# SymbioticLab/Oobleck

Hardware: AMD Instinct MI355X
Metric: tokens/sec (whole node) GPT-2 1F1B (higher is better)
Workload: dtype bf16; 1 GPU; gpt2.yaml GPT-2-small 1F1B, global microbatch 128x1024 tokens, bf16; model=gpt2, global_batch=128, seq_len=1024, parallelism=pp1dp1

## Files before the change

### include/oobleck_stage.h

```cpp
#ifndef OOBLECK_STAGE_H
#define OOBLECK_STAGE_H

#include <stdint.h>

#ifdef __cplusplus
extern "C" {
#endif

enum {
  OB_KIND_EMBED = 0,
  OB_KIND_BLOCK = 1,
  OB_KIND_FINAL = 2
};

typedef struct ob_layer* ob_layer_t;

typedef struct {
  int32_t kind;
  int32_t n_embd;
  int32_t n_head;
  int32_t n_positions;
  int32_t vocab_size;
  int32_t max_batch;
  int32_t seq_len;
// ... 103 lines not shown
int ob_dropout_add_f32(uint64_t seed, int32_t layer_id, int32_t site,
                       uint64_t tick, float p, const void* t, const void* res,
                       void* y, int64_t n, void* stream);
int ob_dropout_add_bf16(uint64_t seed, int32_t layer_id, int32_t site,
                        uint64_t tick, float p, const void* t,
                        const void* res, void* y, int64_t n, void* stream);
int ob_dropout_scale_colsum_f32(uint64_t seed, int32_t layer_id, int32_t site,
                                uint64_t tick, float p, const void* dy,
                                void* dm, void* db, int64_t M, int64_t N,
                                void* stream);
int ob_dropout_scale_colsum_bf16(uint64_t seed, int32_t layer_id, int32_t site,
                                 uint64_t tick, float p, const void* dy,
                                 void* dm, void* db, int64_t M, int64_t N,
                                 void* stream);

int ob_gemm_bf16(int transA, int transB, int64_t M, int64_t N, int64_t K,
                 float alpha, const void* A, int64_t lda,
                 int64_t strideA1, int64_t strideA2,
                 const void* B, int64_t ldb,
                 int64_t strideB1, int64_t strideB2,
                 float beta, void* C, int64_t ldc,
                 int64_t strideC1, int64_t strideC2,
                 int64_t n1, int64_t n2,
                 const void* bias, const void* residual, int out_kind,
                 int splitk, void* stream);

int ob_flash_fwd_nt_bf16(const void* qkv, void* O, void* lse, int64_t B,
                         int64_t Sq, int64_t H, int64_t nh, float scale,
                         void* stream);
int ob_flash_bwd_nt_bf16(const void* qkv, const void* dO, const void* lse,
                         const void* D, void* dqkv, void* dbias_qkv,
                         int64_t B, int64_t Sq, int64_t H, int64_t nh,
                         float scale, void* stream);

int ob_f32_to_bf16(const void* x, void* y, int64_t n, void* stream);
int ob_f32_to_bf16_t(const void* x, void* y, int64_t rows, int64_t cols,
                     void* stream);
int ob_bf16_to_f32(const void* x, void* y, int64_t n, void* stream);

void ob_profile_enable(int on);
void ob_profile_reset(void);
int ob_profile_read(int fam, double* total_ms, long long* count);

const char* ob_last_error(void);

const char* ob_build_arch(void);

#ifdef __cplusplus
}
#endif
#endif
```

### oobleck_amd/_ext.py

```python
from __future__ import annotations

import ctypes
import pathlib

_LIB = None
SO_PATH = pathlib.Path(__file__).resolve().parent / "libob_stage.so"


class ObLayerDesc(ctypes.Structure):
    _fields_ = [
        ("kind", ctypes.c_int32),
        ("n_embd", ctypes.c_int32),
        ("n_head", ctypes.c_int32),
        ("n_positions", ctypes.c_int32),
        ("vocab_size", ctypes.c_int32),
        ("max_batch", ctypes.c_int32),
        ("seq_len", ctypes.c_int32),
        ("n_slots", ctypes.c_int32),
        ("dtype", ctypes.c_int32),
    ]


class ObDropoutDesc(ctypes.Structure):
    _fields_ = [
# ... 82 lines not shown
    lib.ob_flash_fwd_bf16.argtypes = [vp, vp, vp, vp, i64, i64, i64, i64,
                                      f32, vp]
    lib.ob_transpose_bf16_b.argtypes = [vp, vp, i64, i64, i64, i64, i64,
                                        i64, i64, vp]
    lib.ob_layernorm_fwd_bf16.argtypes = [vp, vp, vp, vp, vp, vp, i64, i64,
                                          f32, vp]
    lib.ob_layernorm_bwd_bf16.argtypes = [vp, vp, vp, vp, vp, vp, vp, vp,
                                          i64, i64, i32, vp]
    lib.ob_colsum_bf16.argtypes = [vp, vp, i64, i64, vp]
    lib.ob_layernorm_fwd_copy_bf16.argtypes = [vp, vp, vp, vp, vp, vp, vp,
                                               i64, i64, f32, vp]
    lib.ob_layernorm_bwd_res_bf16.argtypes = [vp, vp, vp, vp, vp, vp, vp, vp,
                                              vp, vp, vp, i64, i64, vp]
    lib.ob_gelu_bwd_colsum_bf16.argtypes = [vp, vp, vp, vp, i64, i64, vp]
    lib.ob_gemm_lt.argtypes = [i32, i32, i64, i64, i64, f32, vp, i64, vp,
                               i64, f32, vp, i64, i32, vp]
    lib.ob_gemm_bf16_nt_8ph.argtypes = [vp, vp, vp, vp, vp, i64, i64, i64,
                                        i64, i64, i64, i64, i64, i64, i64,
                                        i64, i64, i64, i64, f32, f32, i32,
                                        i32, vp, i64]
    lib.ob_profile_enable.argtypes = [i32]
    lib.ob_profile_enable.restype = None
    lib.ob_profile_reset.argtypes = []
    lib.ob_profile_reset.restype = None
    lib.ob_profile_read.argtypes = [i32, ctypes.POINTER(ctypes.c_double),
                                    ctypes.POINTER(ctypes.c_longlong)]
    lib.ob_flash_dsum_bf16.argtypes = [vp, vp, vp, i64, i64, i64, i64, vp]
    lib.ob_flash_bwd_bf16.argtypes = [vp, vp, vp, vp, vp, vp, vp, vp, i64,
                                      i64, i64, i64, f32, vp]
    lib.ob_flash_fwd_nt_bf16.argtypes = [vp, vp, vp, i64, i64, i64, i64,
                                         f32, vp]
    lib.ob_flash_bwd_nt_bf16.argtypes = [vp, vp, vp, vp, vp, vp, i64, i64,
                                         i64, i64, f32, vp]
    return lib


def get_ext(build_if_missing: bool = True) -> ctypes.CDLL:
    global _LIB
    if _LIB is not None:
        return _LIB
    if not SO_PATH.exists():
        if build_if_missing:
            from .build import build
            try:
                build()
            except Exception as e:
                raise RuntimeError(
                    f"oobleck_amd: HIP extension missing and build failed: {e}. "
                    "The hot path has no fallback — run __graft_entry__.build().") from e
        else:
            raise RuntimeError(
                "oobleck_amd: HIP extension libob_stage.so is missing. "
                "The hot path has no fallback — run __graft_entry__.build().")
    _LIB = _configure(ctypes.CDLL(str(SO_PATH)))
    return _LIB


def check(rc: int, what: str = "") -> None:
    if rc != 0:
        err = get_ext().ob_last_error().decode()
        raise RuntimeError(f"oobleck_amd extension error in {what}: {err}")
```

### oobleck_amd/build.py

```python
from __future__ import annotations

import pathlib
import subprocess

PKG_DIR = pathlib.Path(__file__).resolve().parent
SO_PATH = PKG_DIR / "libob_stage.so"
SOURCES = [PKG_DIR / "csrc" / "ob_kernels.hip",
           PKG_DIR / "csrc" / "ob_kernels_bf16.hip",
           PKG_DIR / "csrc" / "ob_flash_bf16.hip",
           PKG_DIR / "csrc" / "ob_blaslt.hip",
           PKG_DIR / "csrc" / "ob_optim.hip",
           PKG_DIR / "csrc" / "ob_dropout.hip",
           PKG_DIR / "csrc" / "ob_layer.hip"]
HEADERS = [PKG_DIR.parent / "include" / "oobleck_stage.h",
           PKG_DIR / "csrc" / "ob_internal.h",
           PKG_DIR / "csrc" / "ob_philox.h"]


def needs_rebuild() -> bool:
    if not SO_PATH.exists():
        return True
    so_mtime = SO_PATH.stat().st_mtime
    return any(p.stat().st_mtime > so_mtime for p in SOURCES + HEADERS)


def build(force: bool = False) -> pathlib.Path:
    if force or needs_rebuild():
        cmd = ["hipcc", "--offload-arch=gfx950", "-O3", "-std=c++17", "-fPIC",
               "-shared"] + [str(s) for s in SOURCES] + \
              ["-L/opt/rocm/lib", "-lhipblaslt", "-o", str(SO_PATH)]
        subprocess.run(cmd, check=True, capture_output=True, text=True)
    return SO_PATH


if __name__ == "__main__":
    print(build(force=True))
```

### oobleck_amd/csrc/ob_flash_bf16.hip

```cpp
#include "ob_internal.h"

#include <cmath>

using f32x16 = __attribute__((ext_vector_type(16))) float;
using bf16x8 = __attribute__((ext_vector_type(8))) __bf16;
using bf16x4 = __attribute__((ext_vector_type(4))) __bf16;

static inline hipStream_t S(void* s) { return reinterpret_cast<hipStream_t>(s); }

__device__ __forceinline__ float bf2f(__bf16 h) { return (float)h; }

__device__ __forceinline__ unsigned bf_bits(__bf16 h) {
  return (unsigned)__builtin_bit_cast(unsigned short, h);
}
__device__ __forceinline__ __bf16 bits_bf(unsigned u) {
  return __builtin_bit_cast(__bf16, (unsigned short)(u & 0xffffu));
}

__device__ __forceinline__ __bf16 bf_extract(const uint4& v, int j) {
  const unsigned word = (j < 2) ? v.x : (j < 4) ? v.y : (j < 6) ? v.z : v.w;
  return bits_bf((j & 1) ? (word >> 16) : word);
}

__device__ __forceinline__ uint4 bf_pack8(const float* v) {
  uint4 o;
  o.x = bf_bits((__bf16)v[0]) | (bf_bits((__bf16)v[1]) << 16);
  o.y = bf_bits((__bf16)v[2]) | (bf_bits((__bf16)v[3]) << 16);
  o.z = bf_bits((__bf16)v[4]) | (bf_bits((__bf16)v[5]) << 16);
  o.w = bf_bits((__bf16)v[6]) | (bf_bits((__bf16)v[7]) << 16);
  return o;
}

__device__ __forceinline__ unsigned bf_pk2(float a, float b) {
// ... 19 lines not shown
  fr.x = x0;
  fr.y = x1;
  fr.z = y0;
  fr.w = y1;
  return __builtin_bit_cast(bf16x8, fr);
}

__device__ __forceinline__ int acc_row(int r, int kh) {
  return (r & 3) + 8 * (r >> 2) + 4 * kh;
}

__device__ __forceinline__ int nt_key(int row) {
  return (((row >> 1) & 1) << 2) | ((row >> 2) & 3);
}
__device__ __forceinline__ int nt_off(int row, int ch) {
  return row * 64 + ((ch ^ nt_key(row)) << 3);
}
__device__ __forceinline__ bf16x8 nt_tr_frag(const __bf16* tile, int lane,
                                             int r0, int dhalf) {
  typedef __attribute__((address_space(3))) bf16x4 lds_bf16x4;
  const int i = lane & 15;
  const int row = r0 + (i >> 2);
  const int ch = 4 * dhalf + 2 * ((lane >> 4) & 1) + ((i >> 1) & 1);
  const int sub = 4 * (i & 1);
  const bf16x4 lo = __builtin_amdgcn_ds_read_tr16_b64_v4bf16(
      (lds_bf16x4*)(tile + nt_off(row, ch) + sub));
  const bf16x4 hi = __builtin_amdgcn_ds_read_tr16_b64_v4bf16(
      (lds_bf16x4*)(tile + nt_off(row + 4, ch) + sub));
  return __builtin_shufflevector(lo, hi, 0, 1, 2, 3, 4, 5, 6, 7);
}

__global__ __launch_bounds__(256, 3) void k_flash_fwd_nt(
    const __bf16* __restrict__ qkv, __bf16* __restrict__ Obase,
    float* __restrict__ lse, int Sq, int H, int nh, float scale) {
  __shared__ __attribute__((aligned(16))) __bf16 kbuf[2][64 * 64];
  __shared__ __attribute__((aligned(16))) __bf16 vbuf[2][64 * 64];
  __shared__ float bcast[128];
  const int z = blockIdx.z;
  const int b = z / nh, h = z % nh;
  const int64_t qoff = (int64_t)b * Sq * 3 * H + h * 64;
  const __bf16* Qp = qkv + qoff;
  const __bf16* Kp = Qp + H;
  const __bf16* Vp = Qp + 2 * H;
  __bf16* Op = Obase + (int64_t)b * Sq * H + h * 64;
  float* lsep = lse + (int64_t)z * Sq;

  const int tid = threadIdx.x;
  const int lane = tid & 63;
  const int w = tid >> 6;
  const int il = lane & 31, kh = lane >> 5;
  const int q0b = blockIdx.x * 128;
  const int q0 = q0b + w * 32;
  const int myq = q0 + il;

  const int sr0 = tid >> 3, sr1 = sr0 + 32, sc = tid & 7;
  const int so0 = nt_off(sr0, sc), so1 = nt_off(sr1, sc);
  auto stage = [&](int buf, int kv0) {
    *reinterpret_cast<bf16x8*>(&kbuf[buf][so0]) =
        *reinterpret_cast<const bf16x8*>(
            Kp + (int64_t)(kv0 + sr0) * 3 * H + sc * 8);
    *reinterpret_cast<bf16x8*>(&kbuf[buf][so1]) =
        *reinterpret_cast<const bf16x8*>(
            Kp + (int64_t)(kv0 + sr1) * 3 * H + sc * 8);
    *reinterpret_cast<bf16x8*>(&vbuf[buf][so0]) =
        *reinterpret_cast<const bf16x8*>(
            Vp + (int64_t)(kv0 + sr0) * 3 * H + sc * 8);
    *reinterpret_cast<bf16x8*>(&vbuf[buf][so1]) =
        *reinterpret_cast<const bf16x8*>(
            Vp + (int64_t)(kv0 + sr1) * 3 * H + sc * 8);
  };

  bf16x8 qf[4];
#pragma unroll
  for (int s = 0; s < 4; ++s)
    qf[s] = *reinterpret_cast<const bf16x8*>(
        Qp + (int64_t)myq * 3 * H + s * 16 + kh * 8);

  const int ntiles = (q0b + 128) / 64;
  stage(0, 0);
  __syncthreads();

  f32x16 o0 = {}, o1 = {};
  float m = -INFINITY, l = 0.f;
  for (int kvt = 0; kvt < ntiles; ++kvt) {
    const int kv0 = kvt * 64;
    if (kvt + 1 < ntiles) stage((kvt + 1) & 1, kv0 + 64);
    const bool active = kv0 <= q0 + 31;
    if (active) {
      const __bf16* kb = kbuf[kvt & 1];
      const __bf16* vb = vbuf[kvt & 1];
      f32x16 sacc0 = {}, sacc1 = {};
#pragma unroll
      for (int s = 0; s < 4; ++s) {
        const int ch = (s * 2 + kh);
        const bf16x8 ka =
            *reinterpret_cast<const bf16x8*>(&kb[nt_off(il, ch)]);
        const bf16x8 kb2 =
            *reinterpret_cast<const bf16x8*>(&kb[nt_off(32 + il, ch)]);
        sacc0 = __builtin_amdgcn_mfma_f32_32x32x16_bf16(ka, qf[s], sacc0, 0,
                                                        0, 0);
        sacc1 = __builtin_amdgcn_mfma_f32_32x32x16_bf16(kb2, qf[s], sacc1,
                                                        0, 0, 0);
      }
      float sv[32];
      if (kv0 + 63 < q0) {
#pragma unroll
        for (int r = 0; r < 16; ++r) {
          sv[r] = sacc0[r] * scale;
          sv[16 + r] = sacc1[r] * scale;
        }
      } else {
#pragma unroll
        for (int r = 0; r < 16; ++r) {
          const int kvr = kv0 + (r & 3) + 8 * (r >> 2) + 4 * kh;
          sv[r] = (kvr <= myq) ? sacc0[r] * scale : -INFINITY;
          sv[16 + r] = (kvr + 32 <= myq) ? sacc1[r] * scale : -INFINITY;
        }
      }
      float mx[8];
#pragma unroll
// ... 27 lines not shown
                   ((ps[4] + ps[5]) + (ps[6] + ps[7]));
      psum += __shfl_xor(psum, 32, 64);
      l += psum;
#pragma unroll
      for (int t = 0; t < 4; ++t) {
        const bf16x8 pa = bf_dance(sv + t * 8);
        const bf16x8 v0f = nt_tr_frag(vb, lane, t * 16 + kh * 8, 0);
        const bf16x8 v1f = nt_tr_frag(vb, lane, t * 16 + kh * 8, 1);
        o0 = __builtin_amdgcn_mfma_f32_32x32x16_bf16(pa, v0f, o0, 0, 0, 0);
        o1 = __builtin_amdgcn_mfma_f32_32x32x16_bf16(pa, v1f, o1, 0, 0, 0);
      }
    }
    __syncthreads();
  }

  if (kh == 0) {
    bcast[w * 32 + il] = 1.f / l;
    lsep[myq] = m + __logf(l);
  }
#pragma unroll
  for (int r = 0; r < 16; ++r) {
    const int row = (r & 3) + 8 * (r >> 2) + 4 * kh;
    const float inv = bcast[w * 32 + row];
    Op[(int64_t)(q0 + row) * H + il] = (__bf16)(o0[r] * inv);
    Op[(int64_t)(q0 + row) * H + 32 + il] = (__bf16)(o1[r] * inv);
  }
}

extern "C" int ob_flash_fwd_nt_bf16(const void* qkv, void* O, void* lse,
                                    int64_t B, int64_t Sq, int64_t H,
                                    int64_t nh, float scale, void* stream) {
  if (H / nh != 64) return ob_fail("flash_fwd_nt: head_dim must be 64");
  if (Sq % 128) return ob_fail("flash_fwd_nt: S must be a multiple of 128");
  dim3 grid((unsigned)(Sq / 128), 1, (unsigned)(B * nh));
  k_flash_fwd_nt<<<grid, 256, 0, S(stream)>>>(
      (const __bf16*)qkv, (__bf16*)O, (float*)lse, (int)Sq, (int)H, (int)nh,
      scale);
  OB_LAUNCH_CHECK();
  return 0;
}

__global__ __launch_bounds__(256, 3) void k_flash_bwd_dkdv_nt(
    const __bf16* __restrict__ qkv, const __bf16* __restrict__ dO,
    const float* __restrict__ lse, const float* __restrict__ D,
    __bf16* __restrict__ dqkv, float* __restrict__ dbias, int Sq, int H,
    int nh, float scale) {
  __shared__ float xch[2][2][32 * 32];
  __shared__ __attribute__((aligned(16))) __bf16 qbuf[2][32 * 64];
  __shared__ __attribute__((aligned(16))) __bf16 obuf[2][32 * 64];
  __shared__ float red[4 * 64];
  const int z = blockIdx.z;
  const int b = z / nh, h = z % nh;
  const int64_t base = (int64_t)b * Sq * 3 * H + h * 64;
  const __bf16* Qp = qkv + base;
  const __bf16* Kp = Qp + H;
  const __bf16* Vp = Qp + 2 * H;
  const __bf16* dOp = dO + (int64_t)b * Sq * H + h * 64;
  const float* lsep = lse + (int64_t)z * Sq;
  const float* Dp = D + (int64_t)z * Sq;

  const int tid = threadIdx.x;
  const int lane = tid & 63;
  const int w = tid >> 6;
  const int pair = w >> 1, role = w & 1;
  const int il = lane & 31, kh = lane >> 5;
  const int kv0 = blockIdx.x * 64 + pair * 32;
  const int mykv = kv0 + il;

  const __bf16* KV = role ? Vp : Kp;
  bf16x8 of[4];
#pragma unroll
  for (int s = 0; s < 4; ++s)
    of[s] = *reinterpret_cast<const bf16x8*>(
        KV + (int64_t)mykv * 3 * H + s * 16 + kh * 8);

  const int srow = tid >> 3, schunk = tid & 7;
  const int so = nt_off(srow, schunk);
  auto stage = [&](int buf, int q0s) {
    *reinterpret_cast<bf16x8*>(&qbuf[buf][so]) =
        *reinterpret_cast<const bf16x8*>(
            Qp + (int64_t)(q0s + srow) * 3 * H + schunk * 8);
    *reinterpret_cast<bf16x8*>(&obuf[buf][so]) =
        *reinterpret_cast<const bf16x8*>(
            dOp + (int64_t)(q0s + srow) * H + schunk * 8);
  };

  f32x16 acc0 = {}, acc1 = {};
  const int nqt = Sq / 32;
  const int qt0 = (blockIdx.x * 64) / 32;
  stage(qt0 & 1, qt0 * 32);
  __syncthreads();

  for (int qt = qt0; qt < nqt; ++qt) {
    const int q0 = qt * 32;
    if (qt + 1 < nqt) stage((qt + 1) & 1, q0 + 32);
    const __bf16* ab = role ? obuf[qt & 1] : qbuf[qt & 1];
    const __bf16* bb = role ? qbuf[qt & 1] : obuf[qt & 1];
    const bf16x8 b00 = nt_tr_frag(bb, lane, kh * 8, 0);
    const bf16x8 b01 = nt_tr_frag(bb, lane, kh * 8, 1);
    const bf16x8 b10 = nt_tr_frag(bb, lane, 16 + kh * 8, 0);
    const bf16x8 b11 = nt_tr_frag(bb, lane, 16 + kh * 8, 1);
    f32x16 own = {};
#pragma unroll
    for (int s = 0; s < 4; ++s) {
      const int ch = s * 2 + kh;
      const bf16x8 af =
          *reinterpret_cast<const bf16x8*>(&ab[nt_off(il, ch)]);
      own = __builtin_amdgcn_mfma_f32_32x32x16_bf16(af, of[s], own, 0, 0,
                                                    0);
    }
    float pv[16];
    float* ptile = xch[qt & 1][pair];
    if (role == 0) {
      const float lse_t = lsep[q0 + il];
#pragma unroll
      for (int r = 0; r < 16; ++r) {
        const int qoff = acc_row(r, kh);
        const bool ok = q0 + qoff >= mykv;
        const float lse_q = __shfl(lse_t, qoff, 64);
        pv[r] = ok ? __expf(own[r] * scale - lse_q) : 0.f;
        ptile[qoff * 32 + il] = pv[r];
      }
    }
    __syncthreads();
    if (role == 1) {
      const float d_t = Dp[q0 + il];
#pragma unroll
      for (int r = 0; r < 16; ++r) {
// ... 12 lines not shown
    }
  }

  __bf16* outp = dqkv + base + (role ? H : 2 * H);
  const float os = role ? scale : 1.f;
#pragma unroll
  for (int r = 0; r < 16; ++r) {
    const int kv = kv0 + acc_row(r, kh);
    outp[(int64_t)kv * 3 * H + il] = (__bf16)(os * acc0[r]);
    outp[(int64_t)kv * 3 * H + 32 + il] = (__bf16)(os * acc1[r]);
  }
  if (dbias) {
    float c0 = 0.f, c1 = 0.f;
#pragma unroll
    for (int r = 0; r < 16; ++r) {
      c0 += os * acc0[r];
      c1 += os * acc1[r];
    }
    c0 += __shfl_xor(c0, 32, 64);
    c1 += __shfl_xor(c1, 32, 64);
    if (kh == 0) {
      red[w * 64 + il] = c0;
      red[w * 64 + 32 + il] = c1;
    }
    __syncthreads();
    if (tid < 128) {
      const int rl = tid >> 6, c = tid & 63;
      atomicAdd(dbias + (rl ? H : 2 * H) + h * 64 + c,
                red[rl * 64 + c] + red[(2 + rl) * 64 + c]);
    }
  }
}

__global__ __launch_bounds__(256, 3) void k_flash_bwd_dq_nt(
    const __bf16* __restrict__ qkv, const __bf16* __restrict__ dO,
    const float* __restrict__ lse, const float* __restrict__ D,
    __bf16* __restrict__ dqkv, float* __restrict__ dbias, int Sq, int H,
    int nh, float scale) {
  __shared__ __attribute__((aligned(16))) __bf16 kbuf[2][64 * 64];
  __shared__ __attribute__((aligned(16))) __bf16 vbuf[2][64 * 64];
  __shared__ float red[4 * 64];
  const int z = blockIdx.z;
  const int b = z / nh, h = z % nh;
  const int64_t base = (int64_t)b * Sq * 3 * H + h * 64;
  const __bf16* Qp = qkv + base;
  const __bf16* Kp = Qp + H;
  const __bf16* Vp = Qp + 2 * H;
  const __bf16* dOp = dO + (int64_t)b * Sq * H + h * 64;
  const float* lsep = lse + (int64_t)z * Sq;
  const float* Dp = D + (int64_t)z * Sq;

  const int tid = threadIdx.x;
  const int lane = tid & 63;
  const int w = tid >> 6;
  const int il = lane & 31, kh = lane >> 5;
  const int q0 = blockIdx.x * 128 + w * 32;
  const int myq = q0 + il;
  const float mylse = lsep[myq];
  const float myD = Dp[myq];

  bf16x8 qf[4], df[4];
#pragma unroll
  for (int s = 0; s < 4; ++s) {
    qf[s] = *reinterpret_cast<const bf16x8*>(
        Qp + (int64_t)myq * 3 * H + s * 16 + kh * 8);
    df[s] = *reinterpret_cast<const bf16x8*>(
        dOp + (int64_t)myq * H + s * 16 + kh * 8);
  }

  const int srow = tid >> 3, schunk = tid & 7;
  const int so0 = nt_off(srow, schunk), so1 = nt_off(srow + 32, schunk);
  auto stage = [&](int buf, int kv0) {
    *reinterpret_cast<bf16x8*>(&kbuf[buf][so0]) =
        *reinterpret_cast<const bf16x8*>(
            Kp + (int64_t)(kv0 + srow) * 3 * H + schunk * 8);
    *reinterpret_cast<bf16x8*>(&kbuf[buf][so1]) =
        *reinterpret_cast<const bf16x8*>(
            Kp + (int64_t)(kv0 + srow + 32) * 3 * H + schunk * 8);
    *reinterpret_cast<bf16x8*>(&vbuf[buf][so0]) =
        *reinterpret_cast<const bf16x8*>(
            Vp + (int64_t)(kv0 + srow) * 3 * H + schunk * 8);
    *reinterpret_cast<bf16x8*>(&vbuf[buf][so1]) =
        *reinterpret_cast<const bf16x8*>(
            Vp + (int64_t)(kv0 + srow + 32) * 3 * H + schunk * 8);
  };

  const int ntiles = (blockIdx.x * 128 + 128) / 64;
  stage(0, 0);
  __syncthreads();

  f32x16 dq0 = {}, dq1 = {};
  for (int kvt = 0; kvt < ntiles; ++kvt) {
    const int kv0 = kvt * 64;
    if (kvt + 1 < ntiles) stage((kvt + 1) & 1, kv0 + 64);
    const bool active = kv0 <= q0 + 31;
    if (active) {
      const __bf16* kb = kbuf[kvt & 1];
      const __bf16* vb = vbuf[kvt & 1];
      f32x16 s0 = {}, s1 = {}, p0 = {}, p1 = {};
#pragma unroll
      for (int s = 0; s < 4; ++s) {
        const int ch = s * 2 + kh;
        const bf16x8 ka =
            *reinterpret_cast<const bf16x8*>(&kb[nt_off(il, ch)]);
        const bf16x8 kb2 =
            *reinterpret_cast<const bf16x8*>(&kb[nt_off(32 + il, ch)]);
        const bf16x8 va =
            *reinterpret_cast<const bf16x8*>(&vb[nt_off(il, ch)]);
        const bf16x8 vb2 =
            *reinterpret_cast<const bf16x8*>(&vb[nt_off(32 + il, ch)]);
        s0 = __builtin_amdgcn_mfma_f32_32x32x16_bf16(ka, qf[s], s0, 0, 0, 0);
        s1 = __builtin_amdgcn_mfma_f32_32x32x16_bf16(kb2, qf[s], s1, 0, 0,
                                                     0);
        p0 = __builtin_amdgcn_mfma_f32_32x32x16_bf16(va, df[s], p0, 0, 0, 0);
        p1 = __builtin_amdgcn_mfma_f32_32x32x16_bf16(vb2, df[s], p1, 0, 0,
                                                     0);
      }
      float dsv[32];
#pragma unroll
      for (int r = 0; r < 16; ++r) {
        const int kv = kv0 + (r & 3) + 8 * (r >> 2) + 4 * kh;
        const bool ok0 = kv <= myq;
        const bool ok1 = kv + 32 <= myq;
        const float pa = ok0 ? __expf(s0[r] * scale - mylse) : 0.f;
        const float pb = ok1 ? __expf(s1[r] * scale - mylse) : 0.f;
        dsv[r] = ok0 ? pa * (p0[r] - myD) : 0.f;
        dsv[16 + r] = ok1 ? pb * (p1[r] - myD) : 0.f;
      }
// ... 5 lines not shown
        dq0 = __builtin_amdgcn_mfma_f32_32x32x16_bf16(da, kt0, dq0, 0, 0, 0);
        dq1 = __builtin_amdgcn_mfma_f32_32x32x16_bf16(da, kt1, dq1, 0, 0, 0);
      }
    }
    __syncthreads();
  }
  __bf16* dQp = dqkv + base;
#pragma unroll
  for (int r = 0; r < 16; ++r) {
    const int q = q0 + (r & 3) + 8 * (r >> 2) + 4 * kh;
    dQp[(int64_t)q * 3 * H + il] = (__bf16)(scale * dq0[r]);
    dQp[(int64_t)q * 3 * H + 32 + il] = (__bf16)(scale * dq1[r]);
  }
  if (dbias) {
    float c0 = 0.f, c1 = 0.f;
#pragma unroll
    for (int r = 0; r < 16; ++r) {
      c0 += scale * dq0[r];
      c1 += scale * dq1[r];
    }
    c0 += __shfl_xor(c0, 32, 64);
    c1 += __shfl_xor(c1, 32, 64);
    if (kh == 0) {
      red[w * 64 + il] = c0;
      red[w * 64 + 32 + il] = c1;
    }
    __syncthreads();
    if (tid < 64)
      atomicAdd(dbias + h * 64 + tid, (red[tid] + red[64 + tid]) +
                                          (red[128 + tid] + red[192 + tid]));
  }
}

extern "C" int ob_flash_bwd_nt_bf16(const void* qkv, const void* dO,
                                    const void* lse, const void* D,
                                    void* dqkv, void* dbias_qkv, int64_t B,
                                    int64_t Sq, int64_t H, int64_t nh,
                                    float scale, void* stream) {
  if (H / nh != 64) return ob_fail("flash_bwd_nt: head_dim must be 64");
  if (Sq % 128) return ob_fail("flash_bwd_nt: S must be a multiple of 128");
  dim3 gridp((unsigned)(Sq / 64), 1, (unsigned)(B * nh));
  k_flash_bwd_dkdv_nt<<<gridp, 256, 0, S(stream)>>>(
      (const __bf16*)qkv, (const __bf16*)dO, (const float*)lse,
      (const float*)D, (__bf16*)dqkv, (float*)dbias_qkv, (int)Sq, (int)H,
      (int)nh, scale);
  OB_LAUNCH_CHECK();
  dim3 grid((unsigned)(Sq / 128), 1, (unsigned)(B * nh));
  k_flash_bwd_dq_nt<<<grid, 256, 0, S(stream)>>>(
      (const __bf16*)qkv, (const __bf16*)dO, (const float*)lse,
      (const float*)D, (__bf16*)dqkv, (float*)dbias_qkv, (int)Sq, (int)H,
      (int)nh, scale);
  OB_LAUNCH_CHECK();
  return 0;
}

__global__ __launch_bounds__(256) void k_flash_dsum(
    const __bf16* __restrict__ O, const __bf16* __restrict__ dO,
    float* __restrict__ D, int Sq, int H, int nh) {
  const int z = blockIdx.z;
  const int b = z / nh, h = z % nh;
  const int row = blockIdx.x * 32 + (threadIdx.x >> 3);
  if (row >= Sq) return;
  const int l8 = threadIdx.x & 7;
  const int64_t off =
      (int64_t)b * Sq * H + (int64_t)row * H + h * 64 + l8 * 8;
  const uint4 ov = *reinterpret_cast<const uint4*>(O + off);
  const uint4 dv = *reinterpret_cast<const uint4*>(dO + off);
  float s = 0.f;
#pragma unroll
  for (int j = 0; j < 8; ++j)
    s += bf2f(bf_extract(ov, j)) * bf2f(bf_extract(dv, j));
#pragma unroll
  for (int o = 4; o > 0; o >>= 1) s += __shfl_down(s, o, 64);
  if (l8 == 0) D[(int64_t)z * Sq + row] = s;
}

extern "C" int ob_flash_dsum_bf16(const void* O, const void* dO, void* D,
                                  int64_t B, int64_t Sq, int64_t H, int64_t nh,
                                  void* stream) {
  dim3 grid((unsigned)((Sq + 31) / 32), 1, (unsigned)(B * nh));
  k_flash_dsum<<<grid, 256, 0, S(stream)>>>(
      (const __bf16*)O, (const __bf16*)dO, (float*)D, (int)Sq, (int)H,
      (int)nh);
  OB_LAUNCH_CHECK();
  return 0;
}
// ... 485 lines not shown
```

### oobleck_amd/csrc/ob_internal.h

```cpp
#pragma once
#include <hip/hip_runtime.h>

#include <cstdarg>
#include <cstdint>
#include <cstdio>

#include "../../include/oobleck_stage.h"

int ob_fail(const char* fmt, ...);

#define OB_HIP(x)                                                     \
  do {                                                                \
    hipError_t e_ = (x);                                              \
    if (e_ != hipSuccess)                                             \
      return ob_fail("%s:%d: %s", __FILE__, __LINE__,                 \
                     hipGetErrorString(e_));                          \
  } while (0)

#define OB_LAUNCH_CHECK()                                             \
  do {                                                                \
    hipError_t e_ = hipGetLastError();                                \
    if (e_ != hipSuccess)                                             \
      return ob_fail("%s:%d: launch: %s", __FILE__, __LINE__,         \
                     hipGetErrorString(e_));                          \
// ... 102 lines not shown
int ob_embed_fwd_bf16(const void* ids, const void* wte, const void* wpe,
                      void* out, int64_t B, int64_t Sq, int64_t H,
                      void* stream);
int ob_embed_bwd_bf16(const void* ids, const void* dout, void* dwte,
                      void* dwpe, int64_t B, int64_t Sq, int64_t H,
                      void* stream);
int ob_ce_fwd_bf16(const void* logits, const void* labels, void* lse,
                   void* loss, int64_t B, int64_t Sq, int64_t V, int64_t ld,
                   void* stream);
int ob_ce_bwd_bf16(void* logits, const void* labels, const void* lse,
                   const void* dloss, int64_t B, int64_t Sq, int64_t V,
                   int64_t ld, void* stream);
int ob_transpose_bf16(const void* in, void* out, int64_t R, int64_t C,
                      void* stream);
int ob_flash_fwd_bf16(const void* qkv, const void* VT, void* O, void* lse,
                      int64_t B, int64_t Sq, int64_t H, int64_t nh,
                      float scale, void* stream);
int ob_transpose_bf16_b(const void* in, void* out, int64_t R, int64_t C,
                        int64_t sIn1, int64_t sIn2, int64_t ldin, int64_t n1,
                        int64_t n2, void* stream);
int ob_flash_dsum_bf16(const void* O, const void* dO, void* D, int64_t B,
                       int64_t Sq, int64_t H, int64_t nh, void* stream);
int ob_flash_bwd_bf16(const void* qkv, const void* QT, const void* KT,
                      const void* dOT, const void* dO, const void* lse,
                      const void* D, void* dqkv, int64_t B, int64_t Sq,
                      int64_t H, int64_t nh, float scale, void* stream);
int ob_flash_fwd_nt_bf16(const void* qkv, void* O, void* lse, int64_t B,
                         int64_t Sq, int64_t H, int64_t nh, float scale,
                         void* stream);
int ob_flash_bwd_nt_bf16(const void* qkv, const void* dO, const void* lse,
                         const void* D, void* dqkv, void* dbias_qkv,
                         int64_t B, int64_t Sq, int64_t H, int64_t nh,
                         float scale, void* stream);
}
extern "C" int ob_gemm_lt(int tA, int tB, int64_t M, int64_t N, int64_t K,
                          float alpha, const void* A, int64_t lda,
                          const void* B, int64_t ldb, float beta, void* C,
                          int64_t ldc, int c_f32, void* stream);
extern "C" int ob_gemm_lt_bias(int tA, int tB, int64_t M, int64_t N,
                               int64_t K, float alpha, const void* A,
                               int64_t lda, const void* B, int64_t ldb,
                               float beta, void* C, int64_t ldc, int c_f32,
                               const void* bias, void* stream);
extern "C" int ob_gemm_lt_bias_res(int tA, int tB, int64_t M, int64_t N,
                                   int64_t K, float alpha, const void* A,
                                   int64_t lda, const void* B, int64_t ldb,
                                   void* C, int64_t ldc, int c_f32,
                                   const void* bias, const void* residual,
                                   void* stream);
extern "C" int ob_gemm_lt_f32(int tA, int tB, int64_t M, int64_t N,
                              int64_t K, float alpha, const void* A,
                              int64_t lda, const void* B, int64_t ldb,
                              float beta, void* C, int64_t ldc,
                              void* stream);
extern "C" int ob_gemm_bf16_nt_8ph(const void* A, const void* B, void* C,
                                   const void* bias, const void* residual,
                                   int64_t M, int64_t N, int64_t K,
                                   int64_t lda, int64_t ldb, int64_t ldc,
                                   int64_t sA1, int64_t sA2, int64_t sB1,
                                   int64_t sB2, int64_t sC1, int64_t sC2,
                                   int64_t n1, int64_t n2, float alpha,
                                   float beta, int out_kind, int splitk,
                                   void* stream, int64_t Mr);
int ob_gemm_bf16_nt_dispatch(const void* A, const void* B, void* C,
                             const void* bias, const void* residual,
                             int64_t M, int64_t N, int64_t K, int64_t lda,
// ... 6 lines not shown
```

### oobleck_amd/csrc/ob_layer.hip

```cpp
#include "ob_internal.h"
#include "ob_philox.h"

#include <cmath>
#include <cstring>
#include <vector>

static inline hipStream_t S(void* s) { return reinterpret_cast<hipStream_t>(s); }
static inline int64_t i64min(int64_t a, int64_t b) { return a < b ? a : b; }
static inline int64_t i64max(int64_t a, int64_t b) { return a > b ? a : b; }


struct Workspace {
  float* dp = nullptr;
  float* bsh1 = nullptr;
  float* bsh2 = nullptr;
  float* dqkv = nullptr;
  float* b4h = nullptr;
  float* t1 = nullptr;
  float* t2 = nullptr;
  float* s1 = nullptr;
  float* s2 = nullptr;
  float* pd_f = nullptr;
  float* pd_b = nullptr;
  float* dm1 = nullptr;
// ... 831 lines not shown
              ob_layernorm_bwd_res_bf16(hmid, p + bp.ln2_w, st + l->o_mean2,
                                        st + l->o_rstd2, DLN, dout, din,
                                        g + bp.ln2_w, g + bp.ln2_b,
                                        dR ? nullptr : g + bp.b_mlpproj,
                                        dR ? nullptr : g + bp.b_attnproj,
                                        BS, H, stream)))
    return 1;
  const __bf16* dap = din;
  if (dR) {
    if (OB_PROF(OB_PF_ELEM, stream,
                ob_drop_scale_colsum(
                    drop_key(l, slot, OB_DROP_RESID_ATTN, l->p_resid), 1, din,
                    g_ws.dm1, g + bp.b_attnproj, BS, H, stream)))
      return 1;
    dap = (const __bf16*)g_ws.dm1;
  }
  OB_SIDE_FENCE(S(stream), g_side.stream);
  if (OB_PROF(OB_PF_GEMM_DX, stream,
              gemm_bf(0, 1, BS, H, H, 1.f, dap, H, 0, 0, sh + l->sh_ap, H, 0,
                      0, DATT, H, 0, 0, 1, 1, nullptr, nullptr, 0, 1,
                      stream)))
    return 1;
  if (OB_PROF(OB_PF_GEMM_DW, side,
              dw_bf16_ws(am, H, dap, H, BS, g + bp.w_attnproj, H, g_ws.s1,
                         g_ws.s2, side)))
    return 1;
  hipEvent_t ev_din_done = side_evt();
  OB_HIP(hipEventRecord(ev_din_done, g_side.stream));
  const bool flash_nt = use_flash(l) && flash_tr();
  if (flash_nt) {
    float* Dbuf = g_ws.t1;
    const float* lseP = st + l->o_p;
    if (OB_PROF(OB_PF_FLASH_BWD, stream,
                ob_flash_dsum_bf16(am, DATT, Dbuf, B, Sq, H, nh, stream)))
      return 1;
    if (OB_PROF(OB_PF_FLASH_BWD, stream,
                ob_flash_bwd_nt_bf16(qkv, DATT, lseP, Dbuf, DQKV,
                                     g + bp.b_qkv, B, Sq, H, nh, scale,
                                     stream)))
      return 1;
  } else if (use_flash(l)) {
    const int64_t BSH = BS * H;
    __bf16* QTw = (__bf16*)g_ws.t1;
    __bf16* KTw = QTw + BSH;
    __bf16* dOTw = KTw + BSH;
    float* Dbuf = g_ws.t1 + (3 * BSH + 1) / 2;
    const float* lseP = st + l->o_p;
    if (OB_PROF(OB_PF_FLASH_BWD, stream,
                ob_transpose_bf16_b(qkv, QTw, Sq, 64, Sq * 3 * H, 64, 3 * H,
                                    B, nh, stream)))
      return 1;
    if (OB_PROF(OB_PF_FLASH_BWD, stream,
                ob_transpose_bf16_b(qkv + H, KTw, Sq, 64, Sq * 3 * H, 64,
                                    3 * H, B, nh, stream)))
      return 1;
    if (OB_PROF(OB_PF_FLASH_BWD, stream,
                ob_transpose_bf16_b(DATT, dOTw, Sq, 64, Sq * H, 64, H, B, nh,
                                    stream)))
      return 1;
    if (OB_PROF(OB_PF_FLASH_BWD, stream,
                ob_flash_dsum_bf16(am, DATT, Dbuf, B, Sq, H, nh, stream)))
      return 1;
    if (OB_PROF(OB_PF_FLASH_BWD, stream,
                ob_flash_bwd_bf16(qkv, QTw, KTw, dOTw, DATT, lseP, Dbuf,
                                  DQKV, B, Sq, H, nh, scale, stream)))
      return 1;
  } else {
    if (OB_PROF(OB_PF_ATTN_MAT, stream,
                gemm_bf(0, 1, Sq, Sq, hd, 1.f, DATT, H, Sq * H, hd,
                        qkv + 2 * H, 3 * H, Sq * 3 * H, hd, DP, Sq,
                        nh * Sq * Sq, Sq * Sq, B, nh, nullptr, nullptr, 0, 1,
                        stream)))
// ... 345 lines not shown
```

Measured before the change: 668,600 tokens/s.

## Fold causal flash tiles for load balance, XCD-swizzle grid, fuse D into dQ

```diff
diff --git a/include/oobleck_stage.h b/include/oobleck_stage.h
--- a/include/oobleck_stage.h
+++ b/include/oobleck_stage.h
@@ -159,6 +159,15 @@
                          const void* D, void* dqkv, void* dbias_qkv,
                          int64_t B, int64_t Sq, int64_t H, int64_t nh,
                          float scale, void* stream);
+int ob_flash_bwd_nt_d_bf16(const void* qkv, const void* O, const void* dO,
+                           const void* lse, void* D_ws, void* dqkv,
+                           void* dbias_qkv, int64_t B, int64_t Sq, int64_t H,
+                           int64_t nh, float scale, void* stream);
+int ob_flash_fold_rows(int64_t kind, int64_t Sq, int64_t block, int64_t unit,
+                       int64_t* row0, int64_t* first_tile, int64_t* n_tiles);
+int64_t ob_flash_fold_grid(int64_t kind, int64_t Sq, int64_t Z);
+int ob_flash_fold_id(int64_t kind, int64_t Sq, int64_t Z, int64_t id,
+                     int64_t* z, int64_t* block);
 
 int ob_f32_to_bf16(const void* x, void* y, int64_t n, void* stream);
 int ob_f32_to_bf16_t(const void* x, void* y, int64_t rows, int64_t cols,
diff --git a/oobleck_amd/_ext.py b/oobleck_amd/_ext.py
--- a/oobleck_amd/_ext.py
+++ b/oobleck_amd/_ext.py
@@ -138,6 +138,13 @@
                                          f32, vp]
     lib.ob_flash_bwd_nt_bf16.argtypes = [vp, vp, vp, vp, vp, vp, i64, i64,
                                          i64, i64, f32, vp]
+    lib.ob_flash_bwd_nt_d_bf16.argtypes = [vp, vp, vp, vp, vp, vp, vp, i64,
+                                           i64, i64, i64, f32, vp]
+    p64 = ctypes.POINTER(ctypes.c_int64)
+    lib.ob_flash_fold_rows.argtypes = [i64, i64, i64, i64, p64, p64, p64]
+    lib.ob_flash_fold_grid.argtypes = [i64, i64, i64]
+    lib.ob_flash_fold_grid.restype = ctypes.c_int64
+    lib.ob_flash_fold_id.argtypes = [i64, i64, i64, i64, p64, p64]
     return lib
 
 
diff --git a/oobleck_amd/build.py b/oobleck_amd/build.py
--- a/oobleck_amd/build.py
+++ b/oobleck_amd/build.py
@@ -14,6 +14,7 @@
            PKG_DIR / "csrc" / "ob_layer.hip"]
 HEADERS = [PKG_DIR.parent / "include" / "oobleck_stage.h",
            PKG_DIR / "csrc" / "ob_internal.h",
+           PKG_DIR / "csrc" / "ob_flash_fold.h",
            PKG_DIR / "csrc" / "ob_philox.h"]
 
 
diff --git a/oobleck_amd/csrc/ob_flash_bf16.hip b/oobleck_amd/csrc/ob_flash_bf16.hip
--- a/oobleck_amd/csrc/ob_flash_bf16.hip
+++ b/oobleck_amd/csrc/ob_flash_bf16.hip
@@ -1,4 +1,5 @@
 #include "ob_internal.h"
+#include "ob_flash_fold.h"
 
 #include <cmath>
 
@@ -84,11 +85,13 @@
 
 __global__ __launch_bounds__(256, 3) void k_flash_fwd_nt(
     const __bf16* __restrict__ qkv, __bf16* __restrict__ Obase,
-    float* __restrict__ lse, int Sq, int H, int nh, float scale) {
+    float* __restrict__ lse, int Sq, int H, int nh, int Z, float scale) {
   __shared__ __attribute__((aligned(16))) __bf16 kbuf[2][64 * 64];
   __shared__ __attribute__((aligned(16))) __bf16 vbuf[2][64 * 64];
   __shared__ float bcast[128];
-  const int z = blockIdx.z;
+  int blk, z;
+  if (!ob_fold_id(blockIdx.x, ob_fold_q_nblk(Sq), Z, &blk, &z))
+    return;
   const int b = z / nh, h = z % nh;
   const int64_t qoff = (int64_t)b * Sq * 3 * H + h * 64;
   const __bf16* Qp = qkv + qoff;
@@ -101,9 +104,9 @@
   const int lane = tid & 63;
   const int w = tid >> 6;
   const int il = lane & 31, kh = lane >> 5;
-  const int q0b = blockIdx.x * 128;
-  const int q0 = q0b + w * 32;
+  const int q0 = ob_fold_q_row0(Sq, blk, w);
   const int myq = q0 + il;
+  const int mytiles = ob_fold_q_wave_tiles(q0);
 
   const int sr0 = tid >> 3, sr1 = sr0 + 32, sc = tid & 7;
   const int so0 = nt_off(sr0, sc), so1 = nt_off(sr1, sc);
@@ -128,7 +131,7 @@
     qf[s] = *reinterpret_cast<const bf16x8*>(
         Qp + (int64_t)myq * 3 * H + s * 16 + kh * 8);
 
-  const int ntiles = (q0b + 128) / 64;
+  const int ntiles = ob_fold_q_block_tiles(Sq, blk);
   stage(0, 0);
   __syncthreads();
 
@@ -137,7 +140,7 @@
   for (int kvt = 0; kvt < ntiles; ++kvt) {
     const int kv0 = kvt * 64;
     if (kvt + 1 < ntiles) stage((kvt + 1) & 1, kv0 + 64);
-    const bool active = kv0 <= q0 + 31;
+    const bool active = kvt < mytiles;
     if (active) {
       const __bf16* kb = kbuf[kvt & 1];
       const __bf16* vb = vbuf[kvt & 1];
@@ -231,10 +234,10 @@
                                     int64_t nh, float scale, void* stream) {
   if (H / nh != 64) return ob_fail("flash_fwd_nt: head_dim must be 64");
   if (Sq % 128) return ob_fail("flash_fwd_nt: S must be a multiple of 128");
-  dim3 grid((unsigned)(Sq / 128), 1, (unsigned)(B * nh));
-  k_flash_fwd_nt<<<grid, 256, 0, S(stream)>>>(
-      (const __bf16*)qkv, (__bf16*)O, (float*)lse, (int)Sq, (int)H, (int)nh,
-      scale);
+  const int Z = (int)(B * nh);
+  k_flash_fwd_nt<<<ob_fold_grid(ob_fold_q_nblk((int)Sq), Z), 256, 0,
+                   S(stream)>>>((const __bf16*)qkv, (__bf16*)O, (float*)lse,
+                                (int)Sq, (int)H, (int)nh, Z, scale);
   OB_LAUNCH_CHECK();
   return 0;
 }
@@ -243,12 +246,14 @@
     const __bf16* __restrict__ qkv, const __bf16* __restrict__ dO,
     const float* __restrict__ lse, const float* __restrict__ D,
     __bf16* __restrict__ dqkv, float* __restrict__ dbias, int Sq, int H,
-    int nh, float scale) {
+    int nh, int Z, float scale) {
   __shared__ float xch[2][2][32 * 32];
   __shared__ __attribute__((aligned(16))) __bf16 qbuf[2][32 * 64];
   __shared__ __attribute__((aligned(16))) __bf16 obuf[2][32 * 64];
   __shared__ float red[4 * 64];
-  const int z = blockIdx.z;
+  int blk, z;
+  if (!ob_fold_id(blockIdx.x, ob_fold_kv_nblk(Sq), Z, &blk, &z))
+    return;
   const int b = z / nh, h = z % nh;
   const int64_t base = (int64_t)b * Sq * 3 * H + h * 64;
   const __bf16* Qp = qkv + base;
@@ -263,8 +268,9 @@
   const int w = tid >> 6;
   const int pair = w >> 1, role = w & 1;
   const int il = lane & 31, kh = lane >> 5;
-  const int kv0 = blockIdx.x * 64 + pair * 32;
+  const int kv0 = ob_fold_kv_row0(Sq, blk, pair);
   const int mykv = kv0 + il;
+  const int myqt0 = ob_fold_kv_pair_first(kv0);
 
   const __bf16* KV = role ? Vp : Kp;
   bf16x8 of[4];
@@ -286,13 +292,17 @@
 
   f32x16 acc0 = {}, acc1 = {};
   const int nqt = Sq / 32;
-  const int qt0 = (blockIdx.x * 64) / 32;
+  const int qt0 = ob_fold_kv_block_first(blk);
   stage(qt0 & 1, qt0 * 32);
   __syncthreads();
 
   for (int qt = qt0; qt < nqt; ++qt) {
     const int q0 = qt * 32;
     if (qt + 1 < nqt) stage((qt + 1) & 1, q0 + 32);
+    if (qt < myqt0) {
+      __syncthreads();
+      continue;
+    }
     const __bf16* ab = role ? obuf[qt & 1] : qbuf[qt & 1];
     const __bf16* bb = role ? qbuf[qt & 1] : obuf[qt & 1];
     const bf16x8 b00 = nt_tr_frag(bb, lane, kh * 8, 0);
@@ -371,15 +381,19 @@
   }
 }
 
+template <bool kFormD>
 __global__ __launch_bounds__(256, 3) void k_flash_bwd_dq_nt(
     const __bf16* __restrict__ qkv, const __bf16* __restrict__ dO,
     const float* __restrict__ lse, const float* __restrict__ D,
+    const __bf16* __restrict__ O, float* __restrict__ Dout,
     __bf16* __restrict__ dqkv, float* __restrict__ dbias, int Sq, int H,
-    int nh, float scale) {
+    int nh, int Z, float scale) {
   __shared__ __attribute__((aligned(16))) __bf16 kbuf[2][64 * 64];
   __shared__ __attribute__((aligned(16))) __bf16 vbuf[2][64 * 64];
   __shared__ float red[4 * 64];
-  const int z = blockIdx.z;
+  int blk, z;
+  if (!ob_fold_id(blockIdx.x, ob_fold_q_nblk(Sq), Z, &blk, &z))
+    return;
   const int b = z / nh, h = z % nh;
   const int64_t base = (int64_t)b * Sq * 3 * H + h * 64;
   const __bf16* Qp = qkv + base;
@@ -387,16 +401,15 @@
   const __bf16* Vp = Qp + 2 * H;
   const __bf16* dOp = dO + (int64_t)b * Sq * H + h * 64;
   const float* lsep = lse + (int64_t)z * Sq;
-  const float* Dp = D + (int64_t)z * Sq;
 
   const int tid = threadIdx.x;
   const int lane = tid & 63;
   const int w = tid >> 6;
   const int il = lane & 31, kh = lane >> 5;
-  const int q0 = blockIdx.x * 128 + w * 32;
+  const int q0 = ob_fold_q_row0(Sq, blk, w);
   const int myq = q0 + il;
+  const int mytiles = ob_fold_q_wave_tiles(q0);
   const float mylse = lsep[myq];
-  const float myD = Dp[myq];
 
   bf16x8 qf[4], df[4];
 #pragma unroll
@@ -406,6 +419,25 @@
     df[s] = *reinterpret_cast<const bf16x8*>(
         dOp + (int64_t)myq * H + s * 16 + kh * 8);
   }
+  float myD;
+  if constexpr (kFormD) {
+    const __bf16* Orow = O + (int64_t)b * Sq * H + h * 64 + (int64_t)myq * H;
+    float cs[4];
+#pragma unroll
+    for (int s = 0; s < 4; ++s) {
+      const bf16x8 ov =
+          *reinterpret_cast<const bf16x8*>(Orow + s * 16 + kh * 8);
+      float c = 0.f;
+#pragma unroll
+      for (int j = 0; j < 8; ++j) c += bf2f(ov[j]) * bf2f(df[s][j]);
+      cs[s] = c;
+    }
+    const float part = (cs[0] + cs[2]) + (cs[1] + cs[3]);
+    myD = part + __shfl_xor(part, 32, 64);
+    if (kh == 0) Dout[(int64_t)z * Sq + myq] = myD;
+  } else {
+    myD = D[(int64_t)z * Sq + myq];
+  }
 
   const int srow = tid >> 3, schunk = tid & 7;
   const int so0 = nt_off(srow, schunk), so1 = nt_off(srow + 32, schunk);
@@ -424,7 +456,7 @@
             Vp + (int64_t)(kv0 + srow + 32) * 3 * H + schunk * 8);
   };
 
-  const int ntiles = (blockIdx.x * 128 + 128) / 64;
+  const int ntiles = ob_fold_q_block_tiles(Sq, blk);
   stage(0, 0);
   __syncthreads();
 
@@ -432,7 +464,7 @@
   for (int kvt = 0; kvt < ntiles; ++kvt) {
     const int kv0 = kvt * 64;
     if (kvt + 1 < ntiles) stage((kvt + 1) & 1, kv0 + 64);
-    const bool active = kv0 <= q0 + 31;
+    const bool active = kvt < mytiles;
     if (active) {
       const __bf16* kb = kbuf[kvt & 1];
       const __bf16* vb = vbuf[kvt & 1];
@@ -504,6 +536,20 @@
   }
 }
 
+static int launch_dkdv_nt(const void* qkv, const void* dO, const void* lse,
+                          const void* D, void* dqkv, void* dbias_qkv,
+                          int64_t B, int64_t Sq, int64_t H, int64_t nh,
+                          float scale, void* stream) {
+  const int Z = (int)(B * nh);
+  k_flash_bwd_dkdv_nt<<<ob_fold_grid(ob_fold_kv_nblk((int)Sq), Z), 256, 0,
+                        S(stream)>>>(
+      (const __bf16*)qkv, (const __bf16*)dO, (const float*)lse,
+      (const float*)D, (__bf16*)dqkv, (float*)dbias_qkv, (int)Sq, (int)H,
+      (int)nh, Z, scale);
+  OB_LAUNCH_CHECK();
+  return 0;
+}
+
 extern "C" int ob_flash_bwd_nt_bf16(const void* qkv, const void* dO,
                                     const void* lse, const void* D,
                                     void* dqkv, void* dbias_qkv, int64_t B,
@@ -511,19 +557,89 @@
                                     float scale, void* stream) {
   if (H / nh != 64) return ob_fail("flash_bwd_nt: head_dim must be 64");
   if (Sq % 128) return ob_fail("flash_bwd_nt: S must be a multiple of 128");
-  dim3 gridp((unsigned)(Sq / 64), 1, (unsigned)(B * nh));
-  k_flash_bwd_dkdv_nt<<<gridp, 256, 0, S(stream)>>>(
-      (const __bf16*)qkv, (const __bf16*)dO, (const float*)lse,
-      (const float*)D, (__bf16*)dqkv, (float*)dbias_qkv, (int)Sq, (int)H,
-      (int)nh, scale);
-  OB_LAUNCH_CHECK();
-  dim3 grid((unsigned)(Sq / 128), 1, (unsigned)(B * nh));
-  k_flash_bwd_dq_nt<<<grid, 256, 0, S(stream)>>>(
-      (const __bf16*)qkv, (const __bf16*)dO, (const float*)lse,
-      (const float*)D, (__bf16*)dqkv, (float*)dbias_qkv, (int)Sq, (int)H,
-      (int)nh, scale);
+  if (launch_dkdv_nt(qkv, dO, lse, D, dqkv, dbias_qkv, B, Sq, H, nh, scale,
+                     stream))
+    return 1;
+  const int Z = (int)(B * nh);
+  k_flash_bwd_dq_nt<false>
+      <<<ob_fold_grid(ob_fold_q_nblk((int)Sq), Z), 256, 0, S(stream)>>>(
+          (const __bf16*)qkv, (const __bf16*)dO, (const float*)lse,
+          (const float*)D, nullptr, nullptr, (__bf16*)dqkv,
+          (float*)dbias_qkv, (int)Sq, (int)H, (int)nh, Z, scale);
   OB_LAUNCH_CHECK();
   return 0;
+}
+
+extern "C" int ob_flash_bwd_nt_d_bf16(const void* qkv, const void* O,
+                                      const void* dO, const void* lse,
+                                      void* D_ws, void* dqkv,
+                                      void* dbias_qkv, int64_t B, int64_t Sq,
+                                      int64_t H, int64_t nh, float scale,
+                                      void* stream) {
+  if (H / nh != 64) return ob_fail("flash_bwd_nt_d: head_dim must be 64");
+  if (Sq % 128) return ob_fail("flash_bwd_nt_d: S must be a multiple of 128");
+  const int Z = (int)(B * nh);
+  k_flash_bwd_dq_nt<true>
+      <<<ob_fold_grid(ob_fold_q_nblk((int)Sq), Z), 256, 0, S(stream)>>>(
+          (const __bf16*)qkv, (const __bf16*)dO, (const float*)lse, nullptr,
+          (const __bf16*)O, (float*)D_ws, (__bf16*)dqkv, (float*)dbias_qkv,
+          (int)Sq, (int)H, (int)nh, Z, scale);
+  OB_LAUNCH_CHECK();
+  return launch_dkdv_nt(qkv, dO, lse, D_ws, dqkv, dbias_qkv, B, Sq, H, nh,
+                        scale, stream);
+}
+
+extern "C" int ob_flash_fold_rows(int64_t kind, int64_t Sq, int64_t block,
+                                  int64_t unit, int64_t* row0,
+                                  int64_t* first_tile, int64_t* n_tiles) {
+  if (Sq <= 0 || Sq % 128) return ob_fail("fold_rows: S must be a multiple of 128");
+  const int S_ = (int)Sq, blk = (int)block;
+  if (kind == OB_FOLD_FWD || kind == OB_FOLD_DQ) {
+    if (blk < 0 || blk >= ob_fold_q_nblk(S_) || unit < -1 || unit > 3)
+      return ob_fail("fold_rows: block/unit out of range");
+    *first_tile = 0;
+    if (unit < 0) {
+      *row0 = -1;
+      *n_tiles = ob_fold_q_block_tiles(S_, blk);
+    } else {
+      *row0 = ob_fold_q_row0(S_, blk, (int)unit);
+      *n_tiles = ob_fold_q_wave_tiles((int)*row0);
+    }
+    return 0;
+  }
+  if (kind == OB_FOLD_DKDV) {
+    if (blk < 0 || blk >= ob_fold_kv_nblk(S_) || unit < -1 || unit > 1)
+      return ob_fail("fold_rows: block/unit out of range");
+    if (unit < 0) {
+      *row0 = -1;
+      *first_tile = ob_fold_kv_block_first(blk);
+    } else {
+      *row0 = ob_fold_kv_row0(S_, blk, (int)unit);
+      *first_tile = ob_fold_kv_pair_first((int)*row0);
+    }
+    *n_tiles = S_ / 32 - *first_tile;
+    return 0;
+  }
+  return ob_fail("fold_rows: unknown kind");
+}
+
+static int fold_nblk(int64_t kind, int64_t Sq) {
+  return kind == OB_FOLD_DKDV ? ob_fold_kv_nblk((int)Sq)
+                              : ob_fold_q_nblk((int)Sq);
+}
+
+extern "C" int64_t ob_flash_fold_grid(int64_t kind, int64_t Sq, int64_t Z) {
+  return (int64_t)ob_fold_grid(fold_nblk(kind, Sq), (int)Z);
+}
+
+extern "C" int ob_flash_fold_id(int64_t kind, int64_t Sq, int64_t Z,
+                                int64_t id, int64_t* z, int64_t* block) {
+  int blk, zz;
+  const bool ok =
+      ob_fold_id((unsigned)id, fold_nblk(kind, Sq), (int)Z, &blk, &zz);
+  *z = zz;
+  *block = blk;
+  return ok ? 1 : 0;
 }
 
 __global__ __launch_bounds__(256) void k_flash_dsum(
diff --git a/oobleck_amd/csrc/ob_flash_fold.h b/oobleck_amd/csrc/ob_flash_fold.h
--- /dev/null
+++ b/oobleck_amd/csrc/ob_flash_fold.h
@@ -0,0 +1,34 @@
+#pragma once
+#include <hip/hip_runtime.h>
+
+#define OB_FOLD_HD __host__ __device__ __forceinline__
+
+enum { OB_FOLD_FWD = 0, OB_FOLD_DQ = 1, OB_FOLD_DKDV = 2 };
+constexpr int OB_FOLD_XCDS = 8;
+
+OB_FOLD_HD int ob_fold_q_nblk(int S) { return S / 128; }
+OB_FOLD_HD int ob_fold_q_row0(int S, int a, int w) {
+  const int n64 = S / 64;
+  return w < 2 ? 64 * a + 32 * w : 64 * (n64 - 1 - a) + 32 * (w - 2);
+}
+OB_FOLD_HD int ob_fold_q_wave_tiles(int q0) { return (q0 + 31) / 64 + 1; }
+OB_FOLD_HD int ob_fold_q_block_tiles(int S, int a) { return S / 64 - a; }
+
+OB_FOLD_HD int ob_fold_kv_nblk(int S) { return S / 64; }
+OB_FOLD_HD int ob_fold_kv_row0(int S, int x, int p) {
+  const int n32 = S / 32;
+  return 32 * (p ? n32 - 1 - x : x);
+}
+OB_FOLD_HD int ob_fold_kv_pair_first(int kv0) { return kv0 / 32; }
+OB_FOLD_HD int ob_fold_kv_block_first(int x) { return x; }
+
+OB_FOLD_HD unsigned ob_fold_grid(int nblk, int Z) {
+  return (unsigned)(OB_FOLD_XCDS * ((Z + OB_FOLD_XCDS - 1) / OB_FOLD_XCDS) *
+                    nblk);
+}
+OB_FOLD_HD bool ob_fold_id(unsigned id, int nblk, int Z, int* blk, int* z) {
+  const int g = (int)(id % OB_FOLD_XCDS), j = (int)(id / OB_FOLD_XCDS);
+  *blk = j % nblk;
+  *z = OB_FOLD_XCDS * (j / nblk) + g;
+  return *z < Z;
+}
diff --git a/oobleck_amd/csrc/ob_internal.h b/oobleck_amd/csrc/ob_internal.h
--- a/oobleck_amd/csrc/ob_internal.h
+++ b/oobleck_amd/csrc/ob_internal.h
@@ -158,6 +158,10 @@
                          const void* D, void* dqkv, void* dbias_qkv,
                          int64_t B, int64_t Sq, int64_t H, int64_t nh,
                          float scale, void* stream);
+int ob_flash_bwd_nt_d_bf16(const void* qkv, const void* O, const void* dO,
+                           const void* lse, void* D_ws, void* dqkv,
+                           void* dbias_qkv, int64_t B, int64_t Sq, int64_t H,
+                           int64_t nh, float scale, void* stream);
 }
 extern "C" int ob_gemm_lt(int tA, int tB, int64_t M, int64_t N, int64_t K,
                           float alpha, const void* A, int64_t lda,
diff --git a/oobleck_amd/csrc/ob_layer.hip b/oobleck_amd/csrc/ob_layer.hip
--- a/oobleck_amd/csrc/ob_layer.hip
+++ b/oobleck_amd/csrc/ob_layer.hip
@@ -887,12 +887,9 @@
     float* Dbuf = g_ws.t1;
     const float* lseP = st + l->o_p;
     if (OB_PROF(OB_PF_FLASH_BWD, stream,
-                ob_flash_dsum_bf16(am, DATT, Dbuf, B, Sq, H, nh, stream)))
-      return 1;
-    if (OB_PROF(OB_PF_FLASH_BWD, stream,
-                ob_flash_bwd_nt_bf16(qkv, DATT, lseP, Dbuf, DQKV,
-                                     g + bp.b_qkv, B, Sq, H, nh, scale,
-                                     stream)))
+                ob_flash_bwd_nt_d_bf16(qkv, am, DATT, lseP, Dbuf, DQKV,
+                                       g + bp.b_qkv, B, Sq, H, nh, scale,
+                                       stream)))
       return 1;
   } else if (use_flash(l)) {
     const int64_t BSH = BS * H;
```

Result: faster. 707,400 tokens/s, median of 6 (+5.8%).
